# kai0511/insider

Hardware: AMD Instinct MI355X
Metric: outer-iterations/sec (masked INSIDER fit, 10000 x 50000, K=30) (higher is better)
Workload: dtype f64

## Files before the change

### insider_amd/csrc/insider_cd_reg.hpp

```cpp
#pragma once

namespace insider {

constexpr int REG_ORDER_OFF = 128;
constexpr int REG3_ORDER_OFF = 124;
static_assert(ORDER_ROW == INSIDER_ORDER_ROW && REG_ORDER_OFF + 8 * 33 <= ORDER_ROW, "a row holds 1 + 32 successor pairs behind the order bytes");
constexpr int REG_BLOCK = INSIDER_REG_BLOCK;
#define REG_STR_(x) #x
#define REG_STR(x) REG_STR_(x)

template <int SLOTS>
struct RegState {
    double y[SLOTS], beta[SLOTS], tau[SLOTS];
};

#define REG_BLOCK_HEAD(KK, HS, BS, IS, IT, DN) REG_ORG(KK) REG_STEP_HEAD(HS, BS, IS, IT, DN)
#define REG_STEP_HEAD(HS, BS, IS, IT, DN)                        \
    "s_lshl_b64 exec, %[lm], " #IT "\n"                          \
    "v_max_f64 %[" DN "], %[" HS "], %[" HS "] clamp\n"          \
    "v_add_f64 %[" DN "], %[" HS "], -%[" DN "]\n"               \
    "v_fma_f64 %[" DN "], -%[" DN "], %[" IS "], %[" BS "]\n"    \
    "s_nop 0\n"                                                  \
    "s_mov_b64 exec, -1\n"
#define REG_PB REG_STR(REG_PBN)
// ... 659 lines not shown
        }
    }
    if ((runm >> lane) & 1ull) {
        my_sweeps = sweep;
#pragma unroll
        for (int u = 0; u < SLOTS; ++u) s_out[64 * u] = S.beta[u];
        if (sweep < max_sweeps) {
            unfinished = true;
#pragma unroll
            for (int u = 0; u < SLOTS; ++u) { hs[u] = S.y[u]; is[u] = S.tau[u]; }
            const float wa = (float)s_acc[0], wb = (float)s_acc[64], wt = (float)((double)W * tol);
            float est = 1048576.0f;
            if (wa > wb && wb > wt) est = (float)W * __logf(wb / wt) / __logf(wa / wb);
            else if (wb <= wt) est = 1.0f;
            key = (int)fminf(fmaxf(est, 1.0f), 1048576.0f);
        } else {
            capped = true;
        }
    }
#pragma unroll
    for (int u = 0; u < SLOTS; ++u) beta[u] = (gene_ok && 16 * u + i < K) ? s_out[64 * u] : 0.0;
    return my_sweeps;
}

struct RegWho {
    int i, j;
    bool gene;
    const double *st;
};

__device__ __forceinline__ RegWho reg_who(const ColArgs &a, int lane)
{
    RegWho w;
    const int row = lane >> 4, slot = blockIdx.x * 4 + row;
    w.i = lane & 15;
    const int count = a.pass_count ? *a.pass_count : a.p;
    w.gene = slot < a.p && slot < count;
    const int sl = w.gene ? slot : 0;
    const int jj = a.gene_perm ? a.gene_perm[sl] : sl;
    w.j = w.gene ? jj : 0;
    w.st = a.stat ? a.stat + (size_t)w.j * a.stat_len : nullptr;
    return w;
}

template <int SLOTS>
__device__ __forceinline__ void reg_load_q(const ColArgs &a, const RegWho &w, double (&q)[SLOTS], double (&Gll)[SLOTS])
{
    const int K = a.K, KP = a.KP;
#pragma unroll
    for (int u = 0; u < SLOTS; ++u) {
        const int c = 16 * u + w.i;
        const bool ok = w.gene && c < K;
        double qv = a.Qfull[(size_t)w.j * KP + c];
        if (w.st) qv -= w.st[stat_index(KP - 1, c)];
        const double d = w.st ? w.st[stat_index(c, c)] : a.RtR[c * KP + c];
        q[u] = ok ? qv : 0.0;
        Gll[u] = ok ? d : 1.0;
    }
}

template <int SLOTS, int KMAX, bool SOLVE>
__global__ void __launch_bounds__(64, reg_waves(KMAX)) k_cd_cols_reg(ColArgs a)
{
    const int lane = threadIdx.x;
    if constexpr (SOLVE && reg_pairs(KMAX)) {
        if (a.code_base) {
            if (blockIdx.x == 0 && lane == 0) {
                a.code_base[0] = reg_code_base<KMAX>();
                a.code_base[1] = reg_pair_base<KMAX>();
            }
// ... 177 lines not shown
```

### insider_amd/csrc/insider_hip.hip

```cpp
#include "insider_kernels.hpp"
#include "insider_posthoc.hpp"
#include "insider_vardecomp.hpp"
#include "insider_sampdecomp.hpp"
#include "insider_levelscores.hpp"
#include "insider_factdecomp.hpp"
#include "insider_outliers.hpp"
#include "insider_neighbors.hpp"
#include "insider_enrich.hpp"
#include "insider_kmeans.hpp"

#include <rccl/rccl.h>

#include <algorithm>
#include <chrono>
#include <cstdlib>
#include <cmath>
#include <cstdio>
#include <cstring>
#include <limits>
#include <memory>
#include <mutex>
#include <atomic>
#include <string>
#include <utility>
// ... 225 lines not shown

struct Workspace {
    static constexpr int EARLY = 3;
    int K = 0, NB = 0, KP = 0, nseg = 1;
    int gram_blocks_p = 0, gram_blocks_n = 0, sc_blocks = 0;
    DevBuf<double> Astack, R, C, RtR, CCt, Qfull, SC, stat, stat_col, gram_part, sc_part, lvl_part, eq, lvl_sum;
    DevBuf<double> fperm;
    DevBuf<double> lvl_zero;
    DevBuf<double> Qheld;
    DevBuf<double> U, Ylvl, wpart, Vlev;
    DevBuf<double> lvl_sum_all;
    DevBuf<double> gram_part2, sc_part2;
    DevBuf<double> wg_part;
    DevBuf<uint8_t> wg_pair;
    DevBuf<double> sse_train, sse_test, b2, b1, loss_buf, stage;
    size_t stage_count = 0;
    DevBuf<int> sweeps, failflag;
    DevBuf<int> sweep_key;
    DevBuf<unsigned long long> sweep_total;
    DevBuf<unsigned> pc4_ticket;
    unsigned pc4_base[2] = {0, 0};
    unsigned long long cd_code_base = 0, cd_pair_base = 0;
    DevBuf<unsigned long long> code_base_dev;
    uint8_t *order = nullptr;
    DevBuf<uint8_t> order_buf[2];
    int order_rows = 0;
    DevBuf<int> gene_perm;
    DevBuf<int> sched_cnt[2], sched_rank;
    DevBuf<uint16_t> sched_bkt;
    int sched_flip = 0;
    DevBuf<double> cd_hsave, cd_isave;
    DevBuf<uint32_t> cd_pass_slot;
    DevBuf<int> cd_pass_perm[2], cd_pass_cnt;
    DevBuf<int> perm_early[EARLY];
    bool have_early[EARLY] = {false, false, false};
    bool have_perm = false;
};

constexpr unsigned EV_SYNC = hipEventDisableTiming | hipEventDisableSystemFence;

struct Streams {
    Stream stream;
    Stream side;
    Stream side2;
    Stream side3;
    Event ev_cd_done, ev_side_done, ev_prep, ev_c_ready;
    Event ev_head;
    std::vector<Event> ev_w;
    Event ev_a_ready, ev_qfull, ev_qheld, ev_tab;

    int create(int n_w)
    {
        HIPCHECK(hipStreamCreate(stream.out()));
        for (Stream *s : {&side, &side2, &side3}) HIPCHECK(hipStreamCreateWithFlags(s->out(), hipStreamNonBlocking));
        for (Event *e : {&ev_prep, &ev_c_ready, &ev_head, &ev_a_ready, &ev_qfull, &ev_qheld, &ev_cd_done, &ev_side_done, &ev_tab})
            HIPCHECK(hipEventCreateWithFlags(e->out(), EV_SYNC));
        ev_w.resize(n_w);
        for (Event &e : ev_w) HIPCHECK(hipEventCreateWithFlags(e.out(), EV_SYNC));
        return INSIDER_OK;
    }
    void synchronize() const
    {
        for (const Stream *s : {&stream, &side, &side2, &side3}) if (*s) (void)hipStreamSynchronize(*s);
    }
};

struct Options {
    int max_sweeps = 1 << 24, order_mode = 0, profile = 0, verbose = 0, cd_variant = 0, force_allreduce = 0;
    int col_factored = 1;
    int row_counts = 1;
    int row_merged = 1;
    int row_gemm = 1;
    int wg_waves = 1024;
    int row_fused = 1;
    int mm_fast = 1;
    int mm_tiles = 0;
    int col_mfma4 = 1;
    int cd_pairs = 1;
    int list_fine = 1;
    int cd_cold_iters = 3, cd_pass_first = 64, cd_pass_ratio = 4;
    double resid_stage_mb = 256.0;
    double vd_stage_kb = 48.0;
    int sd_slabs = 0;
    int ls_slabs = 0;
    double ls_part_mb = 256.0;
    int glm_slabs = 0;
};

struct PostWs {
    DevBuf<double> Ast, U, cp, part, stats, stage, gpart, gram, cpart, gsum, L, dinv, outs;
    DevBuf<int> nz, ints, info;
    DevBuf<double> vin, vtab, vrec;
    DevBuf<double> spart, srec;
    DevBuf<double> lcand, ltab, lpart, lcnt, lout;
    DevBuf<double> fwall, fprod, fbase, frec;
    DevBuf<double> ocs, oz;
    DevBuf<uint32_t> obits;
    DevBuf<int> ogcnt, oscnt, orows, ocols;
    DevBuf<long long> ooffs;
};

}

struct insider_hip_handle {
    std::shared_ptr<const DataSet> ds;
    Streams st;
    Options opt;
    Workspace ws;
    PostWs post;
    bool side_pending = false;
    bool w_ready = false;
    bool qfull_pending = false;
    bool qheld_pending = false;
    int64_t gene_offset = 0;
    int rank = 0, world = 1;
    insider_allreduce_fn allreduce = nullptr;
    void *allreduce_user = nullptr;
    ncclComm_t comm = nullptr;
    std::vector<Event> ev_col, ev_row, ev_cd, ev_test;
    double prof[12] = {0, 0, 0, 0, 0, 0, 0, 0, 0, 0, 0, 0};
    double steady_cd_ms = 0, steady_col_ms = 0;
    int cap_hits = 0, max_gene_sweeps = 0;
    int col_solver = 0, col_eval = 0, col_ridge_fallback = 0;
    int col_stats_kernel = 0, col_stats_tickets = 0, col_stats_blocks = 0;
    int col_q_kernel = 0, mm_rows2_tiles = 0;
    uint64_t row_kernels = 0;
    int vd_path = 0;
    int sd_path = 0, sd_slabs = 0;
    int ls_path = 0, ls_slabs = 0;
    int glm_slabs = 0, glm_form = 0;
    int fd_path = 0;
    int ol_path = 0;

    ~insider_hip_handle()
    {
        if (ds) (void)hipSetDevice(ds->device);
        st.synchronize();
        if (comm) (void)ncclCommDestroy(comm);
    }
};

namespace {

constexpr int PC4_PARTS = 16;
constexpr int MM_FAST_MIN = 16384;
constexpr int MM_SLAB = 128;

enum RowKernel {
    RK_WGEMM4 = 0, RK_WGEMM5, RK_WGEMM6, RK_WGEMM7, RK_WGEMM_CHUNKS, RK_WSYRK, RK_GRAM_SIDE,
    RK_GENE_U_CNT, RK_GENE_U, RK_GENE_UC,
    RK_MERGED_SOLVE, RK_MERGED, RK_MERGED_ZERO, RK_PACK_REDUCE,
    RK_LIST_STATS4, RK_LIST_STATS, RK_LEVEL_PARTIAL, RK_LEVEL_SOLVE, RK_CONT_CD,
    RK_MM_ROWS2, RK_MM_ROWS, RK_MM_REDUCE2_2, RK_MM_REDUCE2_4, RK_MM_REDUCE
};
inline uint64_t rk_bit(RowKernel k) { return 1ull << (int)k; }
inline void row_mark(insider_hip_handle *h, RowKernel k) { h->row_kernels |= rk_bit(k); }
// ... 83 lines not shown
        }
        if ((rc = w.U.alloc((size_t)d.p * round_up(max_L, 2)))) return rc;
        if ((rc = w.Ylvl.alloc(max_L * KP))) return rc;
        if ((rc = w.wpart.alloc((size_t)std::max(d.max_items, 1) * STAT))) return rc;
        if ((rc = w.lvl_sum_all.alloc((size_t)std::max(d.SL, 1) * rec))) return rc;
        if ((rc = w.gram_part2.alloc((size_t)std::max(w.gram_blocks_p, w.gram_blocks_n) * KP * KP))) return rc;
        if ((rc = w.sc_part2.alloc((size_t)w.sc_blocks * d.SL * KP))) return rc;
        if ((rc = w.Vlev.alloc((size_t)d.p * d.SLP))) return rc;
        HIPCHECK(hipMemsetAsync(w.Vlev, 0, (size_t)d.p * d.SLP * sizeof(double), st));
        if ((rc = w.Qheld.alloc((size_t)d.p * KP))) return rc;
    }
    if ((rc = w.eq.alloc((size_t)d.max_L * (KP * KP + KP)))) return rc;
    for (DevBuf<double> *b : {&w.sse_train, &w.sse_test, &w.b2, &w.b1})
        if ((rc = b->alloc((size_t)d.p))) return rc;
    if ((rc = w.loss_buf.alloc(8))) return rc;
    w.stage_count = (size_t)std::max<int64_t>(std::max<int64_t>(d.p, d.n), d.SL) * KP;
    if ((rc = w.stage.alloc(w.stage_count))) return rc;
    if ((rc = w.sweeps.alloc((size_t)d.p))) return rc;
    if ((rc = w.failflag.alloc(4))) return rc;
    if ((rc = w.sweep_total.alloc(256))) return rc;
    if ((rc = w.pc4_ticket.alloc((size_t)(PC4_PARTS + 1) * 32))) return rc;
    HIPCHECK(hipMemsetAsync(w.pc4_ticket, 0, (size_t)(PC4_PARTS + 1) * 32 * sizeof(unsigned), st));
    if ((rc = w.gene_perm.alloc((size_t)d.p))) return rc;
    if ((rc = w.sched_cnt[0].alloc((size_t)SCHED_BUCKETS))) return rc;
    if ((rc = w.sched_cnt[1].alloc((size_t)SCHED_BUCKETS))) return rc;
    if ((rc = w.sched_rank.alloc((size_t)d.p))) return rc;
    if ((rc = w.sched_bkt.alloc((size_t)d.p))) return rc;
    if ((rc = w.sweep_key.alloc((size_t)d.p))) return rc;
    if ((rc = w.cd_hsave.alloc((size_t)d.p * KP))) return rc;
    if ((rc = w.cd_isave.alloc((size_t)d.p * KP))) return rc;
    if ((rc = w.cd_pass_slot.alloc((size_t)d.p))) return rc;
    if ((rc = w.cd_pass_perm[0].alloc((size_t)d.p))) return rc;
    if ((rc = w.cd_pass_perm[1].alloc((size_t)d.p))) return rc;
    if ((rc = w.cd_pass_cnt.alloc((size_t)CD_BUCKETS + 2))) return rc;
    if ((rc = w.code_base_dev.alloc(2))) return rc;
    for (DevBuf<int> &b : w.perm_early)
        if ((rc = b.alloc((size_t)d.p))) return rc;
    HIPCHECK(hipMemsetAsync(w.sched_cnt[0], 0, SCHED_BUCKETS * sizeof(int), st));
    HIPCHECK(hipMemsetAsync(w.sched_cnt[1], 0, SCHED_BUCKETS * sizeof(int), st));
    HIPCHECK(hipMemsetAsync(w.C, 0, (size_t)(std::max<int64_t>(d.p, d.ldp) + 4) * KP * sizeof(double), st));
    HIPCHECK(hipMemsetAsync(w.R, 0, (size_t)d.n * KP * sizeof(double), st));
    HIPCHECK(hipMemsetAsync(w.failflag, 0, 4 * sizeof(int), st));
    w.K = K;
    h->ws = std::move(w);
    return INSIDER_OK;
}

#define NB_DISPATCH(NBV, ...)                                                           \
    switch (NBV) {                                                                      \
        case 1: { constexpr int NB_ = 1; constexpr int WPB_ = 4; __VA_ARGS__; } break;   \
        case 2: { constexpr int NB_ = 2; constexpr int WPB_ = 4; __VA_ARGS__; } break;   \
        case 3: { constexpr int NB_ = 3; constexpr int WPB_ = 2; __VA_ARGS__; } break;   \
        default: { constexpr int NB_ = 4; constexpr int WPB_ = 1; __VA_ARGS__; } break;  \
    }

int launch_list_stats(insider_hip_handle *h, bool cols, int nseg, const double *F, double *stat,
                      const double *base = nullptr, uint64_t *mark = nullptr)
{
    const int units = cols ? (int)h->ds->p : (int)h->ds->n;
    const int64_t f_rows = cols ? h->ds->n : h->ds->p;
    const uint32_t *ptr = cols ? h->ds->col_ptr : h->ds->row_ptr;
    const int *lidx = cols ? h->ds->col_idx : h->ds->row_idx;
    const double *lval = cols ? h->ds->col_val : h->ds->row_val;
    const int64_t items = (int64_t)units * nseg;
    const int NT = (h->ws.K + 4) / 4;
    if (h->opt.list_fine && h->ws.NB == 2 && NT >= 5 && NT <= 8 && h->ws.fperm) {
        hipLaunchKernelGGL(k_tile_perm, dim3(cdiv(f_rows * h->ws.KP, 256)), dim3(256), 0, h->st.stream, F, f_rows, h->ws.KP, h->ws.fperm);
// ... 162 lines not shown
    {
        if (!e0) return INSIDER_OK;
        HIPCHECK(hipEventRecord(e1, h->st.stream));
        into.push_back(std::move(e0));
        into.push_back(std::move(e1));
        return INSIDER_OK;
    }
};

static bool reg3_path(int K, double la) { return K > 32 && K <= 48 && la > 0.0; }

enum ColSolver {
    CS_NONE = 0, CS_RIDGE_REG = 1, CS_RIDGE = 2, CS_CD_REG = 3, CS_CD_REG3 = 4, CS_CD_COLS16 = 5, CS_CD_COLS32 = 6,
    CS_CD_COLS64 = 7, CS_CD_R16_1 = 8, CS_CD_R16_2 = 9, CS_CD_R16_3 = 10
};

static ColSolver cd_solver(int K, double la, int cd_variant)
{
    if (cd_variant == 0 && (K <= 32 || reg3_path(K, la)) && la > 0.0) return K <= 32 ? CS_CD_REG : CS_CD_REG3;
    if (cd_variant == 2 && K <= 16) return CS_CD_R16_1;
    if (cd_variant == 2 && K <= 32) return CS_CD_R16_2;
    if (K <= 16) return CS_CD_COLS16;
    if (K <= 32) return CS_CD_COLS32;
    if (cd_variant != 1 && K <= 48) return CS_CD_R16_3;
    return CS_CD_COLS64;
}

static int launch_cd(ColSolver s, const ColArgs &a, hipStream_t st)
{
    const size_t r16_bytes = (size_t)r16_lds_doubles(a.K) * sizeof(double);
    switch (s) {
        case CS_CD_REG:
        case CS_CD_REG3:
            REG_ANY_DISPATCH(a.K, hipLaunchKernelGGL((k_cd_cols_reg<SL_, KM_, true>), dim3(cdiv(a.p, 4)), dim3(64), 0, st, a));
            break;
        case CS_CD_R16_1: hipLaunchKernelGGL((k_cd_cols_r16<1>), dim3(cdiv(a.p, 4)), dim3(64), r16_bytes, st, a); break;
        case CS_CD_R16_2: hipLaunchKernelGGL((k_cd_cols_r16<2>), dim3(cdiv(a.p, 4)), dim3(64), r16_bytes, st, a); break;
        case CS_CD_R16_3:
            if (int rl = r16_wide_lds(r16_bytes)) return rl;
            hipLaunchKernelGGL((k_cd_cols_r16<3>), dim3(cdiv(a.p, 4)), dim3(64), r16_bytes, st, a);
            break;
        case CS_CD_COLS16: hipLaunchKernelGGL((k_cd_cols<16, 4>), dim3(cdiv(a.p, 16)), dim3(256), 0, st, a); break;
        case CS_CD_COLS32: hipLaunchKernelGGL((k_cd_cols<32, 2>), dim3(cdiv(a.p, 4)), dim3(128), 0, st, a); break;
        case CS_CD_COLS64: hipLaunchKernelGGL((k_cd_cols<64, 1>), dim3((unsigned)a.p), dim3(64), 0, st, a); break;
        default: return fail(INSIDER_ERR_ARG, "not an elastic-net solve kernel");
    }
    KCHECK();
    return INSIDER_OK;
}

static int probe_code_base(int K, unsigned long long *d, hipStream_t st, unsigned long long (&v)[2])
{
    HIPCHECK(hipMemsetAsync(d, 0, 2 * sizeof(unsigned long long), st));
    ColArgs a{};
    a.K = K;
    a.code_base = d;
    REG_DISPATCH(K, hipLaunchKernelGGL((k_cd_cols_reg<SL_, KM_, true>), dim3(1), dim3(64), 0, st, a));
    KCHECK();
    v[0] = v[1] = 0;
    HIPCHECK(hipMemcpyAsync(v, d, sizeof(v), hipMemcpyDeviceToHost, st));
    HIPCHECK(hipStreamSynchronize(st));
    if (!v[0] || !v[1]) return fail(INSIDER_ERR_HIP, "the sweep kernel did not publish the addresses of its code blocks");
    return INSIDER_OK;
}

static int launch_order_table(uint64_t seed, uint32_t iter, int K, int rows, int order_mode, ColSolver s,
                              unsigned long long code_base, unsigned long long pair_base, uint8_t *out, hipStream_t st)
{
    hipLaunchKernelGGL(k_order_table, dim3(cdiv((int64_t)(rows + 1) * 64, 256)), dim3(256), 0, st, seed, iter, K, rows, order_mode,
                       K * 8, reg_kmax(K), (K > 32 && s != CS_CD_REG3) ? 1 : 0, code_base, pair_base, out);
    KCHECK();
    return INSIDER_OK;
}

int ensure_code_base(insider_hip_handle *h, int K)
{
    if (!reg_pairs(reg_kmax(K)) || h->ws.cd_code_base) return INSIDER_OK;
    unsigned long long v[2];
    if (int rc = probe_code_base(K, h->ws.code_base_dev, h->st.stream, v)) return rc;
    h->ws.cd_code_base = v[0];
// ... 245 lines not shown
        a.b1 = h->ws.b1;
        a.sse_test = h->ws.sse_test;
        a.test_from_stats = masked && h->ds->no_na;
        a.sweeps = h->ws.sweeps;
        a.sweep_bins = (timed && solve) ? h->ws.sweep_total : nullptr;
        a.gene_perm = !solve ? nullptr : (early && h->ws.have_early[outer_iter]) ? h->ws.perm_early[outer_iter]
                                       : h->ws.have_perm                         ? h->ws.gene_perm
                                                                              : nullptr;
        a.hsave = h->ws.cd_hsave;
        a.isave = h->ws.cd_isave;
        a.pass_count = nullptr;
        a.resume = 0;
        a.pass_slot = nullptr;
        a.bucket_cnt = nullptr;
        a.cap_hits = solve ? h->ws.failflag + 2 : nullptr;
        a.sched_key = a.sched_cnt = a.sched_rank = nullptr;
        a.sched_bkt = nullptr;
        a.sched_reset = 0;
        const ColSolver cs = cd_solver(h->ws.K, a.cd.la, h->opt.cd_variant);
        if (cs == CS_CD_REG || cs == CS_CD_REG3) {
            if (solve) {
                a.sched_key = h->ws.sweep_key;
                a.sched_cnt = h->ws.sched_cnt[h->ws.sched_flip];
                a.sched_rank = h->ws.sched_rank;
                a.sched_bkt = h->ws.sched_bkt;
                a.sched_reset = (outer_iter < Workspace::EARLY || !h->ws.have_perm) ? 1 : 0;
                fused_bucket = true;
            }
            int limits[16], npass = 0;
            if (solve && outer_iter >= 0 && outer_iter < h->opt.cd_cold_iters && h->opt.cd_pass_first >= 32)
                for (int64_t l = h->opt.cd_pass_first; l < std::min<int64_t>(h->opt.max_sweeps, 4 * (int64_t)INSIDER_PERM_PERIOD) && npass < 16;
                     l *= std::max(h->opt.cd_pass_ratio, 2))
                    limits[npass++] = (int)l;
            int start = 0;
            const int *perm_in = a.gene_perm;
            for (int pass = 0;; ++pass) {
                const int limit = pass < npass ? limits[pass] : 0;
                a.cd.start_sweep = start;
                a.cd.sweep_limit = limit;
                a.pass_slot = npass ? h->ws.cd_pass_slot : nullptr;
                a.bucket_cnt = limit ? h->ws.cd_pass_cnt : nullptr;
                if (limit) HIPCHECK(hipMemsetAsync(h->ws.cd_pass_cnt, 0, CD_BUCKETS * sizeof(int), h->st.stream));
                if (solve) {
                    if ((rc = launch_cd(cs, a, h->st.stream))) return rc;
                    h->col_solver = cs;
                }
                if (!limit) break;
                int *count_out = h->ws.cd_pass_cnt + CD_BUCKETS + (pass & 1);
                hipLaunchKernelGGL(k_pass_scatter, dim3(cdiv(h->ds->p, 256)), dim3(256), 0, h->st.stream,
                                   (const uint32_t *)h->ws.cd_pass_slot, (const int *)h->ws.cd_pass_cnt, perm_in, a.pass_count, (int)h->ds->p,
                                   h->ws.cd_pass_perm[pass & 1], count_out);
                KCHECK();
                perm_in = a.gene_perm = h->ws.cd_pass_perm[pass & 1];
                a.pass_count = count_out;
                a.resume = 1;
                start = limit;
            }
            eval_after = checkpoint != 0;
            eval_args = a;
        } else {
            if ((rc = launch_cd(cs, a, h->st.stream))) return rc;
            h->col_solver = cs;
        }
    }
    if ((rc = t.end(h, h->ev_cd))) return rc;
    if (eval_after) {
        eval_args.gene_perm = nullptr;
        eval_args.pass_count = nullptr;
        eval_args.resume = 0;
        if (h->ws.K <= 32) {
            REG_DISPATCH(h->ws.K, hipLaunchKernelGGL((k_cd_cols_reg<SL_, KM_, false>), dim3(cdiv(h->ds->p, 4)), dim3(64), 0, h->st.stream, eval_args));
            h->col_eval = CS_CD_REG;
        } else {
            const size_t eb = (size_t)r16_lds_doubles(h->ws.K) * sizeof(double);
            if (int rl = r16_wide_lds(eb)) return rl;
            eval_args.mode = COL_EVAL;
            hipLaunchKernelGGL((k_cd_cols_r16<3>), dim3(cdiv(h->ds->p, 4)), dim3(64), eb, h->st.stream, eval_args);
            h->col_eval = CS_CD_R16_3;
        }
        KCHECK();
    }
    if (solve && alpha != 0.0) {
        hipStream_t st = h->st.stream;
        if (side) {
            HIPCHECK(hipEventRecord(h->st.ev_cd_done, h->st.stream));
            HIPCHECK(hipStreamWaitEvent(h->st.side, h->st.ev_cd_done, 0));
            st = h->st.side;
        }
        if ((rc = launch_gene_order(h, h->ws.sweeps, (outer_iter < Workspace::EARLY || !h->ws.have_perm) ? 1 : 0, 0, st, fused_bucket)))
            return rc;
// ... 1169 lines not shown
    if (!h || !unique_id || world < 1 || rank < 0 || rank >= world) return fail(INSIDER_ERR_ARG, "bad communicator arguments");
    if (h->world != world || h->rank != rank) return fail(INSIDER_ERR_ARG, "rank / world differ from insider_hip_set_shard()");
    HIPCHECK(hipSetDevice(h->ds->device));
    if (h->comm) { (void)ncclCommDestroy(h->comm); h->comm = nullptr; }
    ncclUniqueId id;
    std::memcpy(&id, unique_id, sizeof(id));
    const ncclResult_t r = ncclCommInitRank(&h->comm, world, id, rank);
    if (r != ncclSuccess) { h->comm = nullptr; return fail(INSIDER_ERR_COMM, std::string("ncclCommInitRank: ") + ncclGetErrorString(r)); }
    return INSIDER_OK;
}

int insider_hip_set_option(insider_hip_handle *h, const char *name, double value)
{
    if (!h || !name) return fail(INSIDER_ERR_ARG, "null");
    const std::string s(name);
    if (s == "max_sweeps") h->opt.max_sweeps = value < 1 ? 1 : (int)value;
    else if (s == "order_mode") h->opt.order_mode = (int)value;
    else if (s == "profile") h->opt.profile = (int)value;
    else if (s == "verbose") h->opt.verbose = (int)value;
    else if (s == "force_allreduce") h->opt.force_allreduce = (int)value;
    else if (s == "col_factored") h->opt.col_factored = (int)value;
    else if (s == "row_counts") h->opt.row_counts = (int)value;
    else if (s == "row_merged") h->opt.row_merged = (int)value;
    else if (s == "row_gemm_waves") {
        h->opt.wg_waves = std::max(64, (int)value);
        HIPCHECK(hipSetDevice(h->ds->device));
        h->ws = Workspace();
    }
    else if (s == "row_gemm") h->opt.row_gemm = (int)value;
    else if (s == "row_fused") h->opt.row_fused = (int)value;
    else if (s == "cd_cold_iters") h->opt.cd_cold_iters = (int)value;
    else if (s == "cd_pass1") h->opt.cd_pass_first = (int)value;
    else if (s == "cd_pass_ratio") h->opt.cd_pass_ratio = (int)value;
    else if (s == "list_fine") h->opt.list_fine = (int)value;
    else if (s == "mm_fast") h->opt.mm_fast = (int)value;
    else if (s == "mm_tiles") h->opt.mm_tiles = value < 1 ? 0 : (int)value;
    else if (s == "col_mfma4") h->opt.col_mfma4 = (int)value;
    else if (s == "cd_pairs") h->opt.cd_pairs = (int)value;
    else if (s == "resid_stage_mb") h->opt.resid_stage_mb = value;
    else if (s == "vd_stage_kb") h->opt.vd_stage_kb = value;
    else if (s == "ls_slabs") h->opt.ls_slabs = value < 1 ? 0 : (int)std::min(value, 256.0);
    else if (s == "ls_part_mb") h->opt.ls_part_mb = value;
    else if (s == "glm_slabs") h->opt.glm_slabs = value < 1 ? 0 : (int)std::min(value, 64.0);
    else if (s == "sd_slabs") h->opt.sd_slabs = value < 1 ? 0 : (int)std::min(value, 256.0);
    else if (s == "cd_variant") h->opt.cd_variant = (int)value;
    else return fail(INSIDER_ERR_ARG, "unknown option " + s);
    return INSIDER_OK;
}

static int optimize_body(insider_hip_handle *h, double *const *A, double *C, int inc_continuous, int K, double lambda1,
                         double lambda2, double alpha, int tuning, double global_tol, double sub_tol, uint32_t max_iter,
                         uint64_t seed, double *out_train_rmse, double *out_test_rmse, double *out_loss, double *traj,
                         int traj_cap, int *out_traj_rows, int *out_iters)
{
    int rc = check_factor_args(h, A, C, inc_continuous, tuning);
    if (rc) return rc;
    HIPCHECK(hipSetDevice(h->ds->device));
    HIPCHECK(hipStreamSynchronize(h->st.side));
    HIPCHECK(hipStreamSynchronize(h->st.side2));
    HIPCHECK(hipStreamSynchronize(h->st.side3));
    if ((rc = ensure_workspace(h, K))) return rc;
    const auto t_begin = std::chrono::steady_clock::now();
    clear_events(h);
    h->row_kernels = 0;
    h->w_ready = false;
    h->side_pending = false;
    h->qfull_pending = false;
    h->qheld_pending = false;
    const int masked = tuning == 1;
    if ((rc = upload_factors(h, A, C, K))) return rc;

    LossOut lo;
    if ((rc = phase_R(h))) return rc;
    if (masked) if ((rc = launch_col_stats(h, false))) return rc;
    if ((rc = launch_col_solve(h, masked, false, lambda2, alpha, sub_tol, 1, false))) return rc;
    if ((rc = launch_test_sse(h, masked, false))) return rc;
    if ((rc = loss_checkpoint(h, tuning, lambda1, lambda2, alpha, &lo))) return rc;
    double loss = lo.loss, pre_loss, decay = 1.0;
    double train_rmse = lo.train_rmse, test_rmse = lo.test_rmse;
    int trows = 0;
    auto put_traj = [&](double it, double delta, double dec) {
        if (traj && trows < traj_cap) {
            double *t = traj + (size_t)trows * INSIDER_TRAJ_STRIDE;
            t[0] = it; t[1] = lo.train_rmse; t[2] = lo.test_rmse; t[3] = lo.sum_residual / 2; t[4] = lo.row_reg_half;
            t[5] = lo.col_reg_half; t[6] = lo.l1_reg; t[7] = lo.loss; t[8] = delta; t[9] = dec;
            ++trows;
        }
    };
    put_traj(-1, std::numeric_limits<double>::quiet_NaN(), decay);

    uint32_t iter = 0;
    unsigned long long sweeps_total = 0;
    HIPCHECK(hipMemsetAsync(h->ws.sweep_total, 0, 256 * sizeof(unsigned long long), h->st.stream));
    HIPCHECK(hipMemsetAsync(h->ws.failflag + 2, 0, 2 * sizeof(int), h->st.stream));
    if (alpha != 0.0 && !h->ws.have_perm && !h->ws.have_early[0]) {
        hipLaunchKernelGGL(k_yy_key, dim3(cdiv(h->ds->p, 256)), dim3(256), 0, h->st.stream,
                           (const double *)(masked ? h->ds->yy_train : h->ds->yy_all), (int)h->ds->p, h->ws.sweep_key);
// ... 101 lines not shown
        double ms = 0.0;
        int cnt = 0;
        for (size_t i = 10; i + 1 < ev.size(); i += 2) {
            float t = 0;
            if (hipEventElapsedTime(&t, ev[i], ev[i + 1]) == hipSuccess) { ms += t; ++cnt; }
        }
        return cnt ? ms / cnt : 0.0;
    };
    h->steady_cd_ms = tail_mean(h->ev_cd);
    h->steady_col_ms = tail_mean(h->ev_col);
    h->prof[8] = std::chrono::duration<double, std::milli>(t_end - t_begin).count();
    h->prof[9] = (double)std::min<uint64_t>((uint64_t)iter + 1, (uint64_t)max_iter + 1);
    h->prof[10] = (double)sweeps_total;
    h->prof[11] = (masked && use_col_factored(h) ? 1.0 : 0.0) + (use_merged(h, masked) ? 2.0 : 0.0) +
                  (masked && col_stats_path(h) == 2 ? 4.0 : 0.0);
    clear_events(h);
    return INSIDER_OK;
}

int insider_hip_optimize(insider_hip_handle *h, double *const *A, double *C, int inc_continuous, int K, double lambda1,
                         double lambda2, double alpha, int tuning, double global_tol, double sub_tol, uint32_t max_iter,
                         uint64_t seed, double *out_train_rmse, double *out_test_rmse, double *out_loss, double *traj,
                         int traj_cap, int *out_traj_rows, int *out_iters)
{
    const int rc = optimize_body(h, A, C, inc_continuous, K, lambda1, lambda2, alpha, tuning, global_tol, sub_tol, max_iter,
                                 seed, out_train_rmse, out_test_rmse, out_loss, traj, traj_cap, out_traj_rows, out_iters);
    if (rc != INSIDER_OK && h && h->st.stream) {
        const std::string keep = g_err;
        (void)hipSetDevice(h->ds->device);
        (void)hipStreamSynchronize(h->st.stream);
        (void)hipStreamSynchronize(h->st.side);
        (void)hipStreamSynchronize(h->st.side2);
        (void)hipStreamSynchronize(h->st.side3);
        h->side_pending = h->qfull_pending = h->qheld_pending = h->w_ready = false;
        if (h->ws.failflag) (void)hipMemset(h->ws.failflag, 0, 4 * sizeof(int));
        clear_events(h);
        g_err = keep;
    }
    return rc;
}

int insider_hip_optimize_oneshot_ex(const double *X, int64_t n, int64_t p, double *const *A, double *C,
                                    const int32_t *levels, int c, const int32_t *n_levels, const double *ctns, int m,
                                    const uint8_t *M_train, const uint8_t *M_test, int inc_continuous, int K,
                                    double lambda1, double lambda2, double alpha, int tuning, double global_tol,
                                    double sub_tol, uint32_t max_iter, uint64_t seed, int device, double *out_train_rmse,
                                    double *out_test_rmse, double *out_loss)
{
    if (inc_continuous != 0 && inc_continuous != 1)
        return fail(INSIDER_ERR_ARG, "The value of prarameter inc_continuous can only be 0 or 1.");
    if (inc_continuous == 1 && (!ctns || m < 1))
        return fail(INSIDER_ERR_ARG, "inc_continuous = 1 needs ctns_confounder (n x m, m >= 1)");
    insider_hip_handle *h = nullptr;
    int rc = insider_hip_create_ex(X, n, p, levels, c, n_levels, inc_continuous ? ctns : nullptr, inc_continuous ? m : 0,
                                   M_train, M_test, device, &h);
    if (rc) return rc;
    rc = insider_hip_optimize(h, A, C, inc_continuous, K, lambda1, lambda2, alpha, tuning, global_tol, sub_tol, max_iter,
                              seed, out_train_rmse, out_test_rmse, out_loss, nullptr, 0, nullptr, nullptr);
    const std::string keep = g_err;
    insider_hip_destroy(h);
    g_err = keep;
    return rc;
}

int insider_hip_optimize_oneshot(const double *X, int64_t n, int64_t p, double *const *A, double *C,
                                 const int32_t *levels, int c, const int32_t *n_levels, const uint8_t *M_train,
// ... 744 lines not shown

double insider_hip_last_cd_ms(void) { return g_last_cd_ms; }
int insider_hip_last_cd_solver(void) { return g_last_cd_solver; }

int insider_hip_get_sweeps(insider_hip_handle *h, int32_t *out)
{
    if (!h || !out) return fail(INSIDER_ERR_ARG, "null");
    if (!h->ws.sweeps) return fail(INSIDER_ERR_ARG, "no column update has run yet");
    HIPCHECK(hipSetDevice(h->ds->device));
    HIPCHECK(hipStreamSynchronize(h->st.stream));
    HIPCHECK(hipMemcpy(out, h->ws.sweeps, (size_t)h->ds->p * sizeof(int), hipMemcpyDeviceToHost));
    return INSIDER_OK;
}

int insider_hip_get_info(insider_hip_handle *h, const char *name, double *out)
{
    if (!h || !name || !out) return fail(INSIDER_ERR_ARG, "null");
    const std::string s(name);
    const int NB = h->ws.NB;
    if (s == "col_stats_path") *out = col_stats_path(h);
    else if (s == "row_merged") *out = use_merged(h, 1) ? 1.0 : 0.0;
    else if (s == "col_entries") *out = (double)h->ds->col_entries;
    else if (s == "row_entries") *out = (double)h->ds->row_entries;
    else if (s == "data_bytes_shared") *out = (double)h->ds->bytes_shared;
    else if (s == "data_bytes_own") *out = (double)h->ds->bytes_own;
    else if (s == "stat_doubles") *out = NB ? NB * (NB + 1) / 2 * 256.0 : 0.0;
    else if (s == "kp") *out = h->ws.KP;
    else if (s == "pair_count_bytes_per_gene") *out = h->ds->cf_pair_ok ? h->ds->cf.cnt_stride : 0.0;
    else if (s == "lists_bytes") *out = 12.0 * ((double)h->ds->col_entries + (double)h->ds->row_entries);
    else if (s == "cap_hits") *out = h->cap_hits;
    else if (s == "max_gene_sweeps") *out = h->max_gene_sweeps;
    else if (s == "max_sweeps") *out = h->opt.max_sweeps;
    else if (s == "col_solver") *out = h->col_solver;
    else if (s == "col_eval") *out = h->col_eval;
    else if (s == "col_ridge_fallback") *out = h->col_ridge_fallback;
    else if (s == "col_stats_kernel") *out = h->col_stats_kernel;
    else if (s == "col_stats_tickets") *out = h->col_stats_tickets;
    else if (s == "col_stats_blocks") *out = h->col_stats_blocks;
    else if (s == "col_q_kernel") *out = h->col_q_kernel;
    else if (s == "mm_rows2_tiles") *out = h->mm_rows2_tiles;
    else if (s == "n_simd") *out = h->ds->n_simd;
    else if (s == "row_kernels") *out = (double)h->row_kernels;
    else if (s == "cd_ms_steady") *out = h->steady_cd_ms;
    else if (s == "col_stats_ms_steady") *out = h->steady_col_ms;
    else if (s == "ol_path") *out = h->ol_path;
    else if (s == "vd_path") *out = h->vd_path;
    else if (s == "sd_path") *out = h->sd_path;
    else if (s == "ls_path") *out = h->ls_path;
    else if (s == "ls_slabs") *out = h->ls_slabs;
    else if (s == "sd_slabs") *out = h->sd_slabs;
    else if (s == "glm_slabs") *out = h->glm_slabs;
    else if (s == "glm_form") *out = h->glm_form;
    else if (s == "fd_path") *out = h->fd_path;
    else if (s == "col_mfma_per_gene") {
        if (!NB) return fail(INSIDER_ERR_ARG, "no workspace yet: run an update first");
        const int path = col_stats_path(h);
        double v = 0.0;
        if (path == 0) {
            const int NT = (h->ws.K + 4) / 4;
            if (h->opt.list_fine && NB == 2 && NT >= 5 && NT <= 8 && h->ws.fperm)
                v = (double)h->ds->col_entries / (double)std::max<int64_t>(h->ds->p, 1) / 16.0 * (NT * (NT + 1) / 2) / 4.0;
            else
                v = (double)h->ds->col_entries / (double)std::max<int64_t>(h->ds->p, 1) / 4.0 * (NB * (NB + 1) / 2);
        } else
            for (int t = 0; t < h->ds->cf.c; ++t) {
                v += std::ceil(h->ds->cf.L[t] / 4.0) * NB * NB;
// ... 677 lines not shown
```

### insider_amd/csrc/insider_kernels.hpp

```cpp
#pragma once

#include <hip/hip_runtime.h>
#include <stdint.h>

#include "../../include/insider_perm.h"

namespace insider {

typedef double d4 __attribute__((ext_vector_type(4)));
typedef double d2 __attribute__((ext_vector_type(2)));

constexpr int WAVE = 64;
constexpr int CHUNK = 128;

constexpr int LEVEL_CHUNK = 4;
#define INSIDER_ORDER_ROW 448
constexpr int ORDER_ROW = INSIDER_ORDER_ROW;

constexpr int CODE_TRAIN = 1;
constexpr int CODE_TEST = 2;

template <int NB>
struct Geo {
    static constexpr int KP = 16 * NB;
// ... 690 lines not shown
    for (uint32_t o = pos + lane; o < ptr[j + 1]; o += WAVE) { lidx[o] = LIST_PAD; lval[o] = 0.0; if (lflag) lflag[o] = 0; }
}

enum ColMode { COL_EVAL = 0, COL_CD = 1 };

__device__ __forceinline__ int stat_index(int a, int b)
{
    if (a < b) { const int t = a; a = b; b = t; }
    const int bi = a >> 4, bj = b >> 4;
    int i = a & 15, j = b & 15;
    if (bi == bj && i < j) { const int t = i; i = j; j = t; }
    return (bi * (bi + 1) / 2 + bj) * 256 + i * 16 + j;
}

struct ColArgs {
    const double *stat;
    int stat_len;
    int p, K, KP;
    const double *RtR;
    const double *Qfull;
    double *C;
    const double *yy;
    int mode;
    int checkpoint;
    CdParams cd;
    double *sse_train, *b2, *b1;
    double *sse_test;
    int test_from_stats;
    int *sweeps;
    unsigned long long *sweep_bins;
    const int *gene_perm;
    double *hsave, *isave;
    const int *pass_count;
    int resume;
    uint32_t *pass_slot;
    int *bucket_cnt;
    int *cap_hits;
    int *sched_key, *sched_cnt, *sched_rank;
    uint16_t *sched_bkt;
    int sched_reset;
    unsigned long long *code_base = nullptr;
};

constexpr int CD_BUCKETS = 192;
constexpr uint32_t CD_PASS_DONE = 0xFFFFFFFFu;
__device__ __forceinline__ int cd_bucket(int est) { return CD_BUCKETS - 1 - min(CD_BUCKETS - 1, (int)(8.0f * __log2f((float)max(est, 1)))); }

__global__ void __launch_bounds__(256) k_pass_scatter(const uint32_t *__restrict__ pass_slot, const int *__restrict__ bucket_cnt,
                                                      const int *__restrict__ perm_in, const int *__restrict__ count_in, int p,
                                                      int *__restrict__ perm_out, int *__restrict__ count_out)
{
    __shared__ int off[CD_BUCKETS];
    if (threadIdx.x == 0) {
        int run = 0;
        for (int b = 0; b < CD_BUCKETS; ++b) { off[b] = run; run += bucket_cnt[b]; }
        if (blockIdx.x == 0) *count_out = run;
    }
    __syncthreads();
    const int n_in = count_in ? *count_in : p;
    const int slot = blockIdx.x * 256 + threadIdx.x;
    if (slot >= n_in) return;
    const int j = perm_in ? perm_in[slot] : slot;
    const uint32_t v = pass_slot[j];
    if (v != CD_PASS_DONE) perm_out[off[v >> 24] + (int)(v & 0xFFFFFFu)] = j;
}

template <int W, int WPB>
__global__ void __launch_bounds__(WPB * 64) k_cd_cols(ColArgs a)
{
    constexpr int GPW = 64 / W;
    __shared__ double s_G[WPB][GPW][W * W];
    __shared__ int s_ord[WPB][80];
    const int w = threadIdx.x >> 6, lane = threadIdx.x & 63;
    const int grp = lane / W, l = lane & (W - 1);
    const int slot = (blockIdx.x * WPB + w) * GPW + grp;
    const int j = slot < a.p ? (a.gene_perm ? a.gene_perm[slot] : slot) : a.p;
    const int K = a.K, KP = a.KP;
    const bool gene = j < a.p, valid = gene && l < K;
    double *Goff = s_G[w][grp];
    const double *st = (a.stat && gene) ? a.stat + (size_t)j * a.stat_len : nullptr;
    double Gll = 1.0;
    for (int k = 0; k < K; ++k) {
        double v = 0.0;
        if (valid) {
            v = st ? st[stat_index(k, l)] : a.RtR[k * KP + l];
        }
        if (k == l) { Gll = valid ? v : 1.0; v = 0.0; }
        Goff[k * W + l] = v;
    }
    double q = 0.0, beta = 0.0;
    if (valid) {
        q = a.Qfull[(size_t)j * KP + l];
        if (st) q -= st[stat_index(KP - 1, l)];
        beta = a.C[(size_t)j * KP + l];
    }
    wave_sync();
    double g = 0.0;
// ... 787 lines not shown
```

Before: 678.9.

## Split multi-pass gene CD solve into independent chains on parallel streams

```diff
diff --git a/insider_amd/csrc/insider_cd_reg.hpp b/insider_amd/csrc/insider_cd_reg.hpp
--- a/insider_amd/csrc/insider_cd_reg.hpp
+++ b/insider_amd/csrc/insider_cd_reg.hpp
@@ -715,10 +715,10 @@
 __device__ __forceinline__ RegWho reg_who(const ColArgs &a, int lane)
 {
     RegWho w;
-    const int row = lane >> 4, slot = blockIdx.x * 4 + row;
+    const int row = lane >> 4, local = blockIdx.x * 4 + row, slot = a.slot0 + local;
     w.i = lane & 15;
-    const int count = a.pass_count ? *a.pass_count : a.p;
-    w.gene = slot < a.p && slot < count;
+    const int count = a.pass_count ? *a.pass_count : a.slot_n;
+    w.gene = slot < a.p && local < count;
     const int sl = w.gene ? slot : 0;
     const int jj = a.gene_perm ? a.gene_perm[sl] : sl;
     w.j = w.gene ? jj : 0;
diff --git a/insider_amd/csrc/insider_hip.hip b/insider_amd/csrc/insider_hip.hip
--- a/insider_amd/csrc/insider_hip.hip
+++ b/insider_amd/csrc/insider_hip.hip
@@ -281,12 +281,16 @@
     DevBuf<double> cd_hsave, cd_isave;
     DevBuf<uint32_t> cd_pass_slot;
     DevBuf<int> cd_pass_perm[2], cd_pass_cnt;
+    int cd_resident = 0;
     DevBuf<int> perm_early[EARLY];
     bool have_early[EARLY] = {false, false, false};
     bool have_perm = false;
 };
 
 constexpr unsigned EV_SYNC = hipEventDisableTiming | hipEventDisableSystemFence;
+
+constexpr int CD_CHAINS_MAX = 4, CD_CNT_STRIDE = 256;
+static_assert(CD_CNT_STRIDE >= CD_BUCKETS + 2, "a chain's block holds the bucket counters and two list lengths");
 
 struct Streams {
     Stream stream;
@@ -297,6 +301,8 @@
     Event ev_head;
     std::vector<Event> ev_w;
     Event ev_a_ready, ev_qfull, ev_qheld, ev_tab;
+    Stream chain[CD_CHAINS_MAX - 1];
+    Event ev_fork, ev_chain[CD_CHAINS_MAX - 1];
 
     int create(int n_w)
     {
@@ -308,9 +314,23 @@
         for (Event &e : ev_w) HIPCHECK(hipEventCreateWithFlags(e.out(), EV_SYNC));
         return INSIDER_OK;
     }
+    int ensure_chains(int n)
+    {
+        if (!ev_fork) HIPCHECK(hipEventCreateWithFlags(ev_fork.out(), EV_SYNC));
+        for (int i = 0; i < n && i < CD_CHAINS_MAX - 1; ++i) {
+            if (!chain[i]) HIPCHECK(hipStreamCreateWithFlags(chain[i].out(), hipStreamNonBlocking));
+            if (!ev_chain[i]) HIPCHECK(hipEventCreateWithFlags(ev_chain[i].out(), EV_SYNC));
+        }
+        return INSIDER_OK;
+    }
+    void synchronize_chains() const
+    {
+        for (const Stream &s : chain) if (s) (void)hipStreamSynchronize(s);
+    }
     void synchronize() const
     {
         for (const Stream *s : {&stream, &side, &side2, &side3}) if (*s) (void)hipStreamSynchronize(*s);
+        synchronize_chains();
     }
 };
 
@@ -328,6 +348,7 @@
     int cd_pairs = 1;
     int list_fine = 1;
     int cd_cold_iters = 3, cd_pass_first = 64, cd_pass_ratio = 4;
+    int cd_chains = 2, cd_chain_waves = 0;
     double resid_stage_mb = 256.0;
     double vd_stage_kb = 48.0;
     int sd_slabs = 0;
@@ -371,6 +392,7 @@
     double steady_cd_ms = 0, steady_col_ms = 0;
     int cap_hits = 0, max_gene_sweeps = 0;
     int col_solver = 0, col_eval = 0, col_ridge_fallback = 0;
+    int cd_chains_used = 0;
     int col_stats_kernel = 0, col_stats_tickets = 0, col_stats_blocks = 0;
     int col_q_kernel = 0, mm_rows2_tiles = 0;
     uint64_t row_kernels = 0;
@@ -520,7 +542,7 @@
     if ((rc = w.cd_pass_slot.alloc((size_t)d.p))) return rc;
     if ((rc = w.cd_pass_perm[0].alloc((size_t)d.p))) return rc;
     if ((rc = w.cd_pass_perm[1].alloc((size_t)d.p))) return rc;
-    if ((rc = w.cd_pass_cnt.alloc((size_t)CD_BUCKETS + 2))) return rc;
+    if ((rc = w.cd_pass_cnt.alloc((size_t)CD_CHAINS_MAX * CD_CNT_STRIDE))) return rc;
     if ((rc = w.code_base_dev.alloc(2))) return rc;
     for (DevBuf<int> &b : w.perm_early)
         if ((rc = b.alloc((size_t)d.p))) return rc;
@@ -749,7 +771,8 @@
     switch (s) {
         case CS_CD_REG:
         case CS_CD_REG3:
-            REG_ANY_DISPATCH(a.K, hipLaunchKernelGGL((k_cd_cols_reg<SL_, KM_, true>), dim3(cdiv(a.p, 4)), dim3(64), 0, st, a));
+            REG_ANY_DISPATCH(a.K, hipLaunchKernelGGL((k_cd_cols_reg<SL_, KM_, true>), dim3(cdiv(std::min(a.slot_n, a.p - a.slot0), 4)),
+                                                     dim3(64), 0, st, a));
             break;
         case CS_CD_R16_1: hipLaunchKernelGGL((k_cd_cols_r16<1>), dim3(cdiv(a.p, 4)), dim3(64), r16_bytes, st, a); break;
         case CS_CD_R16_2: hipLaunchKernelGGL((k_cd_cols_r16<2>), dim3(cdiv(a.p, 4)), dim3(64), r16_bytes, st, a); break;
@@ -763,6 +786,17 @@
         default: return fail(INSIDER_ERR_ARG, "not an elastic-net solve kernel");
     }
     KCHECK();
+    return INSIDER_OK;
+}
+
+static int cd_resident_waves(insider_hip_handle *h, int *out)
+{
+    if (!h->ws.cd_resident) {
+        int blocks = 0;
+        REG_ANY_DISPATCH(h->ws.K, HIPCHECK(hipOccupancyMaxActiveBlocksPerMultiprocessor(&blocks, (k_cd_cols_reg<SL_, KM_, true>), 64, 0)));
+        h->ws.cd_resident = std::max(1, blocks) * std::max(1, h->ds->n_simd / 4);
+    }
+    *out = h->ws.cd_resident;
     return INSIDER_OK;
 }
 
@@ -1074,30 +1108,62 @@
                 for (int64_t l = h->opt.cd_pass_first; l < std::min<int64_t>(h->opt.max_sweeps, 4 * (int64_t)INSIDER_PERM_PERIOD) && npass < 16;
                      l *= std::max(h->opt.cd_pass_ratio, 2))
                     limits[npass++] = (int)l;
-            int start = 0;
-            const int *perm_in = a.gene_perm;
-            for (int pass = 0;; ++pass) {
-                const int limit = pass < npass ? limits[pass] : 0;
-                a.cd.start_sweep = start;
-                a.cd.sweep_limit = limit;
-                a.pass_slot = npass ? h->ws.cd_pass_slot : nullptr;
-                a.bucket_cnt = limit ? h->ws.cd_pass_cnt : nullptr;
-                if (limit) HIPCHECK(hipMemsetAsync(h->ws.cd_pass_cnt, 0, CD_BUCKETS * sizeof(int), h->st.stream));
-                if (solve) {
-                    if ((rc = launch_cd(cs, a, h->st.stream))) return rc;
-                    h->col_solver = cs;
+            auto run_chain = [&](ColArgs c, hipStream_t st, int slot0, int n, int *cnt) -> int {
+                int start = 0;
+                const int *perm_in = c.gene_perm;
+                c.slot0 = slot0;
+                c.slot_n = n;
+                for (int pass = 0;; ++pass) {
+                    const int limit = pass < npass ? limits[pass] : 0;
+                    c.cd.start_sweep = start;
+                    c.cd.sweep_limit = limit;
+                    c.pass_slot = npass ? h->ws.cd_pass_slot : nullptr;
+                    c.bucket_cnt = limit ? cnt : nullptr;
+                    if (limit) HIPCHECK(hipMemsetAsync(cnt, 0, CD_BUCKETS * sizeof(int), st));
+                    if (solve)
+                        if (int rl = launch_cd(cs, c, st)) return rl;
+                    if (!limit) break;
+                    int *count_out = cnt + CD_BUCKETS + (pass & 1);
+                    hipLaunchKernelGGL(k_pass_scatter, dim3(cdiv(n, 256)), dim3(256), 0, st, (const uint32_t *)h->ws.cd_pass_slot,
+                                       (const int *)cnt, perm_in, c.pass_count, n, h->ws.cd_pass_perm[pass & 1], count_out, slot0);
+                    KCHECK();
+                    perm_in = c.gene_perm = h->ws.cd_pass_perm[pass & 1];
+                    c.pass_count = count_out;
+                    c.resume = 1;
+                    start = limit;
                 }
-                if (!limit) break;
-                int *count_out = h->ws.cd_pass_cnt + CD_BUCKETS + (pass & 1);
-                hipLaunchKernelGGL(k_pass_scatter, dim3(cdiv(h->ds->p, 256)), dim3(256), 0, h->st.stream,
-                                   (const uint32_t *)h->ws.cd_pass_slot, (const int *)h->ws.cd_pass_cnt, perm_in, a.pass_count, (int)h->ds->p,
-                                   h->ws.cd_pass_perm[pass & 1], count_out);
-                KCHECK();
-                perm_in = a.gene_perm = h->ws.cd_pass_perm[pass & 1];
-                a.pass_count = count_out;
-                a.resume = 1;
-                start = limit;
+                return INSIDER_OK;
+            };
+            const int waves = (int)cdiv(h->ds->p, 4);
+            int nchain = 1, chunk_waves = waves;
+            if (npass && h->opt.cd_chains > 1) {
+                const int max_chains = std::min(h->opt.cd_chains, CD_CHAINS_MAX);
+                chunk_waves = h->opt.cd_chain_waves;
+                if (chunk_waves < 1) {
+                    int resident = 0;
+                    if ((rc = cd_resident_waves(h, &resident))) return rc;
+                    chunk_waves = waves <= resident ? waves : (int)cdiv((int64_t)4 * resident, 3);
+                }
+                nchain = (int)std::min<int64_t>(max_chains, cdiv(waves, chunk_waves));
             }
+            if (nchain <= 1) {
+                if ((rc = run_chain(a, h->st.stream, 0, (int)h->ds->p, h->ws.cd_pass_cnt))) return rc;
+            } else {
+                if ((rc = h->st.ensure_chains(nchain - 1))) return rc;
+                HIPCHECK(hipEventRecord(h->st.ev_fork, h->st.stream));
+                if ((rc = run_chain(a, h->st.stream, 0, chunk_waves * 4, h->ws.cd_pass_cnt))) return rc;
+                for (int ch = 1; ch < nchain; ++ch) {
+                    const int slot0 = ch * chunk_waves * 4;
+                    const int n = ch + 1 < nchain ? chunk_waves * 4 : (int)h->ds->p - slot0;
+                    const hipStream_t cst = h->st.chain[ch - 1];
+                    HIPCHECK(hipStreamWaitEvent(cst, h->st.ev_fork, 0));
+                    if ((rc = run_chain(a, cst, slot0, n, h->ws.cd_pass_cnt + ch * CD_CNT_STRIDE))) return rc;
+                    HIPCHECK(hipEventRecord(h->st.ev_chain[ch - 1], cst));
+                }
+                for (int ch = 1; ch < nchain; ++ch) HIPCHECK(hipStreamWaitEvent(h->st.stream, h->st.ev_chain[ch - 1], 0));
+            }
+            h->cd_chains_used = std::max(h->cd_chains_used, nchain);
+            if (solve) h->col_solver = cs;
             eval_after = checkpoint != 0;
             eval_args = a;
         } else {
@@ -2333,6 +2399,8 @@
     else if (s == "cd_cold_iters") h->opt.cd_cold_iters = (int)value;
     else if (s == "cd_pass1") h->opt.cd_pass_first = (int)value;
     else if (s == "cd_pass_ratio") h->opt.cd_pass_ratio = (int)value;
+    else if (s == "cd_chains") h->opt.cd_chains = (int)value;
+    else if (s == "cd_chain_waves") h->opt.cd_chain_waves = value < 1 ? 0 : (int)value;
     else if (s == "list_fine") h->opt.list_fine = (int)value;
     else if (s == "mm_fast") h->opt.mm_fast = (int)value;
     else if (s == "mm_tiles") h->opt.mm_tiles = value < 1 ? 0 : (int)value;
@@ -2360,10 +2428,12 @@
     HIPCHECK(hipStreamSynchronize(h->st.side));
     HIPCHECK(hipStreamSynchronize(h->st.side2));
     HIPCHECK(hipStreamSynchronize(h->st.side3));
+    h->st.synchronize_chains();
     if ((rc = ensure_workspace(h, K))) return rc;
     const auto t_begin = std::chrono::steady_clock::now();
     clear_events(h);
     h->row_kernels = 0;
+    h->cd_chains_used = 0;
     h->w_ready = false;
     h->side_pending = false;
     h->qfull_pending = false;
@@ -2531,6 +2601,7 @@
         (void)hipStreamSynchronize(h->st.side);
         (void)hipStreamSynchronize(h->st.side2);
         (void)hipStreamSynchronize(h->st.side3);
+        h->st.synchronize_chains();
         h->side_pending = h->qfull_pending = h->qheld_pending = h->w_ready = false;
         if (h->ws.failflag) (void)hipMemset(h->ws.failflag, 0, 4 * sizeof(int));
         clear_events(h);
@@ -3341,6 +3412,7 @@
     else if (s == "max_gene_sweeps") *out = h->max_gene_sweeps;
     else if (s == "max_sweeps") *out = h->opt.max_sweeps;
     else if (s == "col_solver") *out = h->col_solver;
+    else if (s == "cd_chains_used") *out = h->cd_chains_used;
     else if (s == "col_eval") *out = h->col_eval;
     else if (s == "col_ridge_fallback") *out = h->col_ridge_fallback;
     else if (s == "col_stats_kernel") *out = h->col_stats_kernel;
diff --git a/insider_amd/csrc/insider_kernels.hpp b/insider_amd/csrc/insider_kernels.hpp
--- a/insider_amd/csrc/insider_kernels.hpp
+++ b/insider_amd/csrc/insider_kernels.hpp
@@ -746,6 +746,7 @@
     const int *gene_perm;
     double *hsave, *isave;
     const int *pass_count;
+    int slot0 = 0, slot_n = 0x7fffffff;
     int resume;
     uint32_t *pass_slot;
     int *bucket_cnt;
@@ -762,7 +763,7 @@
 
 __global__ void __launch_bounds__(256) k_pass_scatter(const uint32_t *__restrict__ pass_slot, const int *__restrict__ bucket_cnt,
                                                       const int *__restrict__ perm_in, const int *__restrict__ count_in, int p,
-                                                      int *__restrict__ perm_out, int *__restrict__ count_out)
+                                                      int *__restrict__ perm_out, int *__restrict__ count_out, int slot0)
 {
     __shared__ int off[CD_BUCKETS];
     if (threadIdx.x == 0) {
@@ -774,9 +775,9 @@
     const int n_in = count_in ? *count_in : p;
     const int slot = blockIdx.x * 256 + threadIdx.x;
     if (slot >= n_in) return;
-    const int j = perm_in ? perm_in[slot] : slot;
+    const int j = perm_in ? perm_in[slot0 + slot] : slot0 + slot;
     const uint32_t v = pass_slot[j];
-    if (v != CD_PASS_DONE) perm_out[off[v >> 24] + (int)(v & 0xFFFFFFu)] = j;
+    if (v != CD_PASS_DONE) perm_out[slot0 + off[v >> 24] + (int)(v & 0xFFFFFFu)] = j;
 }
 
 template <int W, int WPB>
```

New measurement: 678.0. About the same (-0.1%).
